# uncbiag/OAI_analysis_2

Hardware: NVIDIA B200
Metric: knee volumes/sec (seg+ICON reg+warp) (higher is better)
Workload: dtype fp16 operands / fp32 accumulate (tcgen05 kind::f16), the full-resolution decoder layers read fp16 hi+lo activations (dc2: skip input only; dc1); fp32 registration; fp64 warp coordinates

## Files before the change

include/oai_b200.h:

```cpp
#ifndef OAI_B200_H_
#define OAI_B200_H_

#include <stddef.h>
#include <stdint.h>

#if defined(__GNUC__)
#define OAI_API __attribute__((visibility("default")))
#else
#define OAI_API
#endif

#ifdef __cplusplus
extern "C" {
#endif

OAI_API const char* oai_last_error(void);
OAI_API int oai_version(void);
OAI_API long long oai_launch_count(void);


OAI_API int oai_conv3d_igemm(const void* src0, int c0, const void* src1, int c1, int NT, int D, int H, int W,
                     const void* wpack, size_t wpack_bytes, const float* bias, int cout, int pointwise, int relu,
                     int ab_format, void* out, long long obase, long long osN, long long osD, long long osH,
                     long long osW, int flags, void* stream);

OAI_API int oai_conv3d_igemm_region(const void* src0, int c0, const void* src1, int c1, int NT, int D, int H, int W,
                                    const void* wpack, size_t wpack_bytes, const float* bias, int cout, int pointwise,
                                    int relu, int ab_format, void* out, long long obase, long long osN, long long osD,
                                    long long osH, long long osW, int flags, const int* region, void* stream);

OAI_API int oai_pack_convt2_weights(const float* w, int cout, int cin, int D, int H, int W, int ab_format, void* dst,
                                    size_t dst_bytes);
OAI_API int oai_convt2_igemm(const void* src, int cin, int NT, int D, int H, int W, const void* wpack,
                             size_t wpack_bytes, const float* bias, int cout, int relu, int ab_format, void* out,
                             const int* region, void* stream);

OAI_API int oai_conv3d_igemm_head(const void* src0, int c0, const void* src1, int c1, int NT, int D, int H, int W,
                                  const void* wpack, size_t wpack_bytes, const float* bias, int ab_format, int ncls,
                                  const float* head_w, const float* head_b, float* out, const int* vol_dims,
                                  const int* geom, int tile0, const int* crop_zyx, int out_mode, int flags,
                                  void* stream);

OAI_API int oai_conv3d_igemm_plan(int D, int H, int W, int c0, int c1, int cout, int pointwise, int flags, int* plan);

OAI_API int oai_pack_conv_weights(const float* w, int cout, int c0, int c1, int D, int H, int W, int pointwise, int ab_format,
                          int flags, void* dst, size_t dst_bytes);

OAI_API int oai_conv3d_igemm_plan_ex(int D, int H, int W, int c0, int c1, int cout, int pointwise, int terms, int flags,
                                     int* plan);
OAI_API int oai_pack_conv_weights_ex(const float* w, int cout, int c0, int c1, int D, int H, int W, int pointwise,
                                     int terms, int ab_format, int flags, void* dst, size_t dst_bytes);
OAI_API int oai_conv3d_igemm_ex(const void* src0, int c0, const void* src1, int c1, int in_split, int NT, int D, int H,
                                int W, const void* wpack, size_t wpack_bytes, const float* bias, int cout,
                                int pointwise, int relu, int ab_format, int terms, void* out, int out_split, int flags,
                                const int* region, void* stream);

OAI_API int oai_conv_overflow_count(long long* count, int reset, void* stream);

// ... 193 lines not shown
```

oai_analysis_2_b200/csrc/api_conv.cu:

```cuda
#include "../../include/oai_b200.h"
#include "api_common.h"
#include "conv_api.h"
#include "conv_igemm.cuh"

#include <cuda_bf16.h>
#include <cuda_fp16.h>

#include <cstring>
#include <vector>

namespace oai {

cudaError_t conv_igemm_launch(const ConvIgemmParams& p, const CUtensorMap& tm0, const CUtensorMap& tm1, int num_sms,
                              cudaStream_t stream);
cudaError_t conv_overflow_count(unsigned int* count, bool reset, cudaStream_t stream);

namespace {

constexpr int kFlagForcePerTap = 1;
constexpr int kFlagBaseOffFormula = 2;
constexpr int kFlagForceKd1 = 4;
constexpr int kFlagNoFastPath = 8;
constexpr int kFlagWideN = 16;
constexpr int kFlagWideRows = 32;
constexpr int kFlagNoPingPong = 128;
constexpr int kFlagOneKhRow = 64;
constexpr size_t kSmemBudget = 232448 - 1024 - 48 * 8 - 2112 - 2048;

struct Chunk {
  int src, cc, wsel, dup;
};

struct Plan {
  int mode, kd_per_block, R, Rd, up_groups, nhalf, cph, nblk, nch, k16, row_bytes, TW, TH, n_wbuf, n_astage;
  int nkh;
  int pingpong;
  int stationary;
  uint32_t wblock_bytes, astage_bytes, astage_stride;
  Chunk chunks[kMaxChunks];
};

inline bool split_src(int terms, int src) {
  return terms == 2 || terms == 3 || (terms == 4 && src == 1) || (terms == 5 && src == 0);
}

int build_chunks(const ConvSpec& s, Plan* pl) {
  int n = 0;
  const int cs[2] = {s.c0, s.c1};
  for (int src = 0; src < 2; ++src) {
// ... 274 lines not shown
                const int v = ck.cc + j;
                if (v >= (ck.dup ? 2 * csrc : csrc)) break;
                const int ci = cbase + (ck.dup ? v % csrc : v);
                const uint16_t h = wrow[static_cast<size_t>(ci) * ktaps + tap];
                memcpy(blk + swz_off(r, j, pl.row_bytes), &h, 2);
              }
            }
          }
      }
  return 0;
}

int conv_run(const ConvSpec& s, const ConvLaunch& a, cudaStream_t st) {
  const int D = s.D, H = s.H, W = s.W, c0 = s.c0, c1 = s.c1, cout = s.cout;
  const bool kh_shared = (s.flags & kConvFlagKhShared) != 0;
  int d_lo = 0, d_cnt = D, h_lo = 0, h_cnt = H, w_lo = 0, w_cnt = W;
  if (a.region) {
    d_lo = a.region[0]; d_cnt = a.region[1]; h_lo = a.region[2]; h_cnt = a.region[3];
    OAI_REQUIRE(d_lo >= 0 && d_cnt >= 1 && d_lo + d_cnt <= D && h_lo >= 0 && h_cnt >= 1 && h_lo + h_cnt <= H,
                "conv: region [%d,+%d)x[%d,+%d) outside %dx%d", d_lo, d_cnt, h_lo, h_cnt, D, H);
  }
  if (a.w_cnt) {
    w_lo = a.w_lo; w_cnt = a.w_cnt;
    OAI_REQUIRE(kh_shared, "conv: a w range needs a layer packed for kh-shared mode");
    OAI_REQUIRE(w_lo >= 0 && w_cnt >= 1 && w_lo + w_cnt <= W, "conv: w range [%d,+%d) outside W=%d", w_lo, w_cnt, W);
  }
  int tw = 32, ntile = 0;
  if (kh_shared)
    for (int t = 32; t >= 8; t /= 2) {
      if (t > W || 128 / t > H) continue;
      const int n = ((w_cnt + t - 1) / t) * ((h_cnt + 128 / t - 1) / (128 / t));
      if (ntile == 0 || n < ntile) { ntile = n; tw = t; }
    }
  Plan pl;
  if (make_plan(s, &pl, d_cnt, tw)) return 1;
  int tile_h_lo = h_lo, nph = (h_cnt + pl.TH - 1) / pl.TH, npw = (w_cnt + pl.TW - 1) / pl.TW;
  if (!kh_shared) {
    tile_h_lo = h_lo / pl.TH * pl.TH;
    nph = (h_lo + h_cnt + pl.TH - 1) / pl.TH - h_lo / pl.TH;
    npw = W / pl.TW;
  }
  const HeadFuse* head = a.head;
  OAI_REQUIRE(a.src0 && a.wpack && a.bias, "conv: null pointer");
  OAI_REQUIRE(!head || (pl.cph == 64 && pl.nhalf == 1), "conv head: the fused head needs a 64-channel layer");
  OAI_REQUIRE((c1 == 0) == (a.src1 == nullptr), "conv: src1/c1 mismatch");
  const size_t need = plan_wpack_bytes(pl);
  OAI_REQUIRE(a.wpack_bytes == need, "conv: packed weights are %zu bytes, geometry needs %zu", a.wpack_bytes, need);
// ... 8 lines not shown
  p.TW = pl.TW; p.TH = pl.TH; p.R = pl.R;
  p.cout = pl.cph; p.nhalf = pl.nhalf;
  p.nchunks = pl.nch; p.k16_steps = pl.k16; p.row_bytes = pl.row_bytes;
  for (int c = 0; c < pl.nch; ++c) {
    p.chunk_src[c] = static_cast<uint8_t>(pl.chunks[c].src);
    p.chunk_cc[c] = static_cast<uint16_t>(pl.chunks[c].cc);
  }
  p.mode = pl.mode; p.kd_per_block = pl.kd_per_block; p.nblk = pl.nblk / pl.nkh;
  p.wblock_bytes = pl.wblock_bytes * pl.nkh; p.n_wbuf = pl.n_wbuf; p.n_astage = pl.n_astage;
  p.nkh = pl.nkh;
  p.acc_pingpong = pl.pingpong;
  p.w_stationary = pl.stationary;
  p.astage_bytes = pl.astage_bytes; p.astage_stride = pl.astage_stride;
  p.ab_format = s.fmt; p.relu = a.relu;
  p.base_off_mode = (s.flags & kFlagBaseOffFormula) ? 1 : 0;
  p.no_fast_path = (s.flags & kFlagNoFastPath) ? 1 : 0;
  p.wpack = static_cast<const uint8_t*>(a.wpack);
  p.bias = a.bias;
  p.out = a.out;
  p.obase = a.obase; p.osN = a.osN; p.osD = a.osD; p.osH = a.osH; p.osW = a.osW;
  p.out_split = a.out_split; p.out_lo_off = a.out_lo_off;
  p.d_lo = d_lo; p.d_cnt = d_cnt; p.h_lo = tile_h_lo; p.nph = nph; p.w_lo = kh_shared ? w_lo : 0; p.npw = npw;
  p.Rd = pl.Rd; p.up_groups = pl.up_groups;
  p.nunits = a.NT * ((d_cnt + pl.Rd - 1) / pl.Rd) * (nph * npw) * pl.up_groups * pl.nhalf;
  if (pl.mode == kModeUp2) {
    const long long vox = a.osW / 2;
    for (int t = 0; t < 8; ++t)
      p.tap_off[t] = ((static_cast<long long>(t >> 2) * 2 * H + ((t >> 1) & 1)) * 2 * W + (t & 1)) * vox;
  }
  if (head) p.head = *head;

  OAI_REQUIRE(pl.mode != kModeUp2 || (c1 == 0 && !head), "conv: up2 mode takes one source and no fused head");
  const int bw = pl.mode == kModeRowShared ? 130 : pl.TW;
  const int bh = pl.mode == kModeKhShared ? pl.TH + 2 : pl.TH * pl.nkh;
  CUtensorMap tm0, tm1;
  if (make_act_tmap(&tm0, a.src0, s.split0 ? 2 * c0 : c0, W, H, D, a.NT, bw, bh, s.fmt, pl.row_bytes)) return 1;
  if (a.src1) {
    if (make_act_tmap(&tm1, a.src1, s.split1 ? 2 * c1 : c1, W, H, D, a.NT, bw, bh, s.fmt)) return 1;
  } else {
    tm1 = tm0;
  }
  ProfEntry* pe = nullptr;
  if (g_prof_on) {
    if (g_prof_used == g_prof.size()) {
      ProfEntry ne;
      if (cudaEventCreate(&ne.a) != cudaSuccess || cudaEventCreate(&ne.b) != cudaSuccess)
        return fail("conv profile: cannot create events");
// ... 174 lines not shown
  if (int rc = check_cuda(cudaEventSynchronize(g_prof[i].b), "conv profile: event sync")) return rc;
  float t = 0;
  if (int rc = check_cuda(cudaEventElapsedTime(&t, g_prof[i].a, g_prof[i].b), "conv profile: elapsed")) return rc;
  if (ms) *ms = t;
  if (flops) *flops = g_prof[i].flops;
  if (exec_flops) *exec_flops = g_prof[i].exec_flops;
  return 0;
}


extern "C" int oai_pack_convt2_weights(const float* w, int cout, int cin, int D, int H, int W, int ab_format,
                                       void* dst, size_t dst_bytes) {
  return conv_pack_weights(spec_of(D, H, W, cin, 0, cout, 2, ab_format, 0), w, dst, dst_bytes);
}

extern "C" int oai_convt2_igemm(const void* src, int cin, int NT, int D, int H, int W, const void* wpack,
                                size_t wpack_bytes, const float* bias, int cout, int relu, int ab_format, void* out,
                                const int* region, void* stream) {
  OAI_REQUIRE(out != nullptr, "convt2: null output");
  const long long c = cout;
  return conv_common(src, cin, nullptr, 0, NT, D, H, W, wpack, wpack_bytes, bias, cout, 2, relu, ab_format, out, 0,
                     8ll * D * H * W * c, 8ll * H * W * c, 4ll * W * c, 2 * c, 0, nullptr, region, stream);
}
```

oai_analysis_2_b200/csrc/conv_api.h:

```cpp
#pragma once
#include <cstddef>
#include <cuda_runtime.h>

#include "conv_igemm.cuh"

namespace oai {

constexpr int kConvFlagKhShared = 256;

struct ConvSpec {
  int D, H, W;
  int c0, c1;
  int split0, split1;
  int cout;
  int kind;
  int terms;
  int fmt;
  int flags;
};

struct ConvLaunch {
  const void* src0;
  const void* src1;
  int NT;
  const void* wpack;
  size_t wpack_bytes;
  const float* bias;
  int relu;
  void* out;
  long long obase, osN, osD, osH, osW;
  int out_split;
// ... 25 lines not shown
```

oai_analysis_2_b200/csrc/conv_igemm.cu:

```cuda
#include "conv_igemm.cuh"
#include "ptx.cuh"

#include <cuda_bf16.h>
#include <cuda_fp16.h>

namespace oai {

namespace {

constexpr int kThreads = 384;
constexpr int kEpiGroups = 2;
constexpr int kTmemCols = 512;

__device__ unsigned int g_fp16_overflow = 0;

struct BlockInfo {
  int c, kh, kw, kdlo, nkd;
  int ns;
};

__device__ __forceinline__ BlockInfo decode_block(const ConvIgemmParams& p, int b) {
  BlockInfo bi;
  if (p.mode == kModeRowShared) {
    bi.c = p.nkh == 3 ? b : b / 3;
// ... 26 lines not shown
  } else {
    bi.c = b;
    bi.kh = 1;
    bi.kw = 1;
    bi.kdlo = 1;
    bi.nkd = 1;
  }
  bi.ns = (p.mode == kModeUp2) ? p.R : bi.nkd;
  return bi;
}

struct UnitInfo {
  int n, d0, h0, w0, nh;
  int tg;
  int rd;
  int ra;
};

__device__ __forceinline__ UnitInfo decode_unit(const ConvIgemmParams& p, int u) {
  UnitInfo ui;
  const int npw = p.npw;
  const int np = npw * p.nph, ndg = (p.d_cnt + p.Rd - 1) / p.Rd;
  if (p.w_stationary) {
    const int per_key = np * ndg * p.NT;
    const int key = u / per_key;
    u -= key * per_key;
    ui.tg = key % p.up_groups;
    ui.nh = key / p.up_groups;
  } else {
    ui.nh = u % p.nhalf;
    u /= p.nhalf;
    ui.tg = u % p.up_groups;
    u /= p.up_groups;
  }
  const int patch = u % np;
  u /= np;
  ui.d0 = p.d_lo + (u % ndg) * p.Rd;
  ui.n = u / ndg;
  ui.h0 = min(p.h_lo + (patch / npw) * p.TH, p.H - p.TH);
  ui.w0 = min(p.w_lo + (patch % npw) * p.TW, p.W - p.TW);
  ui.rd = min(p.Rd, p.d_lo + p.d_cnt - ui.d0);
  ui.ra = (p.mode == kModeUp2) ? p.R : ui.rd;
  return ui;
}

template <int FMT>
__device__ __forceinline__ uint32_t pack2(float a, float b) {
  if (FMT == 0) {
    __half2 h = __floats2half2_rn(a, b);
// ... 1 lines not shown
  }
  __nv_bfloat162 h = __floats2bfloat162_rn(a, b);
  return *reinterpret_cast<uint32_t*>(&h);
}

__device__ __forceinline__ void st_global_256(void* p, const uint32_t* v) {
  asm volatile("st.global.v8.b32 [%0], {%1,%2,%3,%4,%5,%6,%7,%8};" ::"l"(p), "r"(v[0]), "r"(v[1]), "r"(v[2]), "r"(v[3]),
               "r"(v[4]), "r"(v[5]), "r"(v[6]), "r"(v[7])
               : "memory");
}

template <int FMT>
__device__ __forceinline__ uint32_t pack2_residual(float a, float b, uint32_t hi) {
  if (FMT == 0) {
    const float2 h = __half22float2(*reinterpret_cast<const __half2*>(&hi));
    return pack2<FMT>(a - h.x, b - h.y);
  }
  const float2 h = __bfloat1622float2(*reinterpret_cast<const __nv_bfloat162*>(&hi));
  return pack2<FMT>(a - h.x, b - h.y);
}

template <int FMT, bool RELU, bool SPLIT>
__device__ __forceinline__ void epi_store_chunk(uint32_t (&v)[32], uint32_t sbias, uint16_t* dst, long long lo_off,
                                                float& amax) {
  uint32_t o[16];
#pragma unroll
  for (int i = 0; i < 8; ++i) {
    const float4 b4 = lds_f4(sbias + 16 * i);
    float x0 = __uint_as_float(v[4 * i]) + b4.x, x1 = __uint_as_float(v[4 * i + 1]) + b4.y;
    float x2 = __uint_as_float(v[4 * i + 2]) + b4.z, x3 = __uint_as_float(v[4 * i + 3]) + b4.w;
    if (RELU) {
      x0 = fmaxf(x0, 0.f); x1 = fmaxf(x1, 0.f); x2 = fmaxf(x2, 0.f); x3 = fmaxf(x3, 0.f);
    }
    amax = fmaxf(amax, fmaxf(fmaxf(fabsf(x0), fabsf(x1)), fmaxf(fabsf(x2), fabsf(x3))));
    o[2 * i] = pack2<FMT>(x0, x1);
    o[2 * i + 1] = pack2<FMT>(x2, x3);
    if (SPLIT) {
      v[4 * i] = __float_as_uint(x0); v[4 * i + 1] = __float_as_uint(x1);
      v[4 * i + 2] = __float_as_uint(x2); v[4 * i + 3] = __float_as_uint(x3);
    }
  }
  st_global_256(dst, o);
  st_global_256(dst + 16, o + 8);
  if (SPLIT) {
#pragma unroll
    for (int i = 0; i < 16; ++i)
      o[i] = pack2_residual<FMT>(__uint_as_float(v[2 * i]), __uint_as_float(v[2 * i + 1]), o[i]);
    st_global_256(dst + lo_off, o);
    st_global_256(dst + lo_off + 16, o + 8);
  }
}

template <int FMT, bool RELU, bool SPLIT>
__device__ __forceinline__ void epi_store_acc(uint32_t t_acc, int nb, uint32_t sbias, uint16_t* dst, long long lo_off,
                                              uint64_t* acc_empty_bar, int lane, float& amax) {
  for (int j = 0; j < nb; ++j) {
    uint32_t v[32];
    tmem_ld_32x32(t_acc + j * 32, v);
    tmem_ld_wait();
    if (j + 1 == nb) {
      tc_fence_before();
      __syncwarp();
      if (lane == 0) mbar_arrive(acc_empty_bar);
    }
    epi_store_chunk<FMT, RELU, SPLIT>(v, sbias + j * 128, dst + j * 32, lo_off, amax);
  }
}

template <int NC>
__device__ __forceinline__ void head_dot(const uint32_t (&v)[32], uint32_t sbias, uint32_t sw, float (&acc)[8],
                                         int ncls = NC) {
#pragma unroll
  for (int i = 0; i < 8; ++i) {
    const float4 b4 = lds_f4(sbias + 16 * i);
    const float f0 = fmaxf(__uint_as_float(v[4 * i]) + b4.x, 0.f), f1 = fmaxf(__uint_as_float(v[4 * i + 1]) + b4.y, 0.f);
    const float f2 = fmaxf(__uint_as_float(v[4 * i + 2]) + b4.z, 0.f), f3 = fmaxf(__uint_as_float(v[4 * i + 3]) + b4.w, 0.f);
#pragma unroll
    for (int k = 0; k < NC; ++k)
      if (k < ncls) {
        const float4 w4 = lds_f4(sw + k * 256 + 16 * i);
        acc[k] = fmaf(f3, w4.w, fmaf(f2, w4.z, fmaf(f1, w4.y, fmaf(f0, w4.x, acc[k]))));
      }
  }
}


struct IssueConsts {
  uint32_t kw_step, b_kw, desc_hi32, idesc_1, idesc_step, tap16, cout;
// ... 358 lines not shown
    const int per_rt = max(1, 256 / p.cout);
#define OAI_ISSUE(NKW, K16N, PER) \
  mma_issuer_fast<NKW, K16N, PER, 1>(p, tmem_base, abuf, wbuf, wstride, full_a, empty_a, full_w, empty_w, acc_full, acc_empty)
#define OAI_ISSUE_GENERAL() \
  mma_issuer_general(p, tmem_base, abuf, wbuf, wstride, full_a, empty_a, full_w, empty_w, acc_full, acc_empty)
    if (general) OAI_ISSUE_GENERAL();
    else if (nkw_rt == 3 && p.k16_steps == 4 && per_rt == 4) OAI_ISSUE(3, 4, 4);
    else if (nkw_rt == 3 && p.k16_steps == 2 && per_rt == 4 && p.nkh == 3)
      mma_issuer_fast<3, 2, 4, 3>(p, tmem_base, abuf, wbuf, wstride, full_a, empty_a, full_w, empty_w, acc_full, acc_empty);
    else if (nkw_rt == 3 && p.k16_steps == 2 && per_rt == 4) OAI_ISSUE(3, 2, 4);
    else if (nkw_rt == 1 && p.k16_steps == 4 && per_rt == 4) OAI_ISSUE(1, 4, 4);
    else if (nkw_rt == 1 && p.k16_steps == 4 && per_rt == 2) OAI_ISSUE(1, 4, 2);
    else if (nkw_rt == 1 && p.k16_steps == 4 && per_rt == 1) OAI_ISSUE(1, 4, 1);
    else OAI_ISSUE_GENERAL();
#undef OAI_ISSUE_GENERAL
#undef OAI_ISSUE
  } else if (warp >= 4) {
    const int q = warp & 3;
    const int eg = (warp - 4) >> 2;
    const int epi_variant = (p.ab_format ? 4 : 0) + (p.out_split ? 2 : 0) + (p.relu ? 1 : 0);
    const uint32_t s_bias_addr = smem_u32(s_bias), s_head_addr = smem_u32(s_head);
    const int m = q * 32 + lane;
    const int th = m / p.TW, tw = m % p.TW;
    uint32_t ub0 = 0, ub1 = 0;
    int half = 0;
    const uint32_t tmem_base0 = tmem_base;
    uint64_t* const acc_full0 = acc_full;
    uint64_t* const acc_empty0 = acc_empty;
    uint16_t* out = reinterpret_cast<uint16_t*>(p.out);
    float amax = 0.f;
    for (int u = blockIdx.x; u < p.nunits; u += gridDim.x) {
      const UnitInfo ui = decode_unit(p, u);
      const int ab = half * p.R;
      const uint32_t tmem_base = tmem_base0 + static_cast<uint32_t>(ab * p.cout);
      uint64_t* const acc_full = acc_full0 + ab;
      uint64_t* const acc_empty = acc_empty0 + ab;
      const int this_half = half;
      const uint32_t use_bits = this_half ? ub1 : ub0;
      if (p.acc_pingpong) half ^= 1;
      const long long off0 = p.obase + ui.n * p.osN + (ui.h0 + th) * p.osH + (ui.w0 + tw) * p.osW +
                             static_cast<long long>(ui.nh) * p.cout;
      for (int a = 0; a < ui.ra; ++a) {
        if (((ab + a) % kEpiGroups) != eg) continue;
        mbar_wait(&acc_full[a], (use_bits >> a) & 1u, 600 + a);
        tc_fence_after();
        if (p.head.enabled) {
          const HeadFuse& hd = p.head;
          const int z = ui.d0 + a - hd.od, y = ui.h0 + th - hd.oh, x = ui.w0 + tw - hd.ow;
          const bool row_in = z >= 0 && z < hd.ed;
          const bool mine = row_in && y >= 0 && y < hd.eh && x >= 0 && x < hd.ew;
          if (__any_sync(0xffffffffu, mine)) {
            float acc[8];
#pragma unroll
            for (int k = 0; k < 8; ++k) acc[k] = 0.f;
            for (int j = 0; j < 2; ++j) {
              uint32_t v[32];
              tmem_ld_32x32(tmem_base + (static_cast<uint32_t>(q * 32) << 16) +
                                static_cast<uint32_t>(a * p.cout + j * 32), v);
              tmem_ld_wait();
              const uint32_t sbj = s_bias_addr + static_cast<uint32_t>(ui.nh * p.cout + j * 32) * 4u;
              const uint32_t swj = s_head_addr + static_cast<uint32_t>(j * 32) * 4u;
              switch (hd.ncls) {
                case 1: head_dot<1>(v, sbj, swj, acc); break;
                case 2: head_dot<2>(v, sbj, swj, acc); break;
// ... 12 lines not shown
                const size_t o = (static_cast<size_t>(gz) * hd.VH + gy) * hd.VW + gx;
                const size_t cls_stride = static_cast<size_t>(hd.VD) * hd.VH * hd.VW;
#pragma unroll
                for (int k = 0; k < 8; ++k) {
                  if (k >= hd.ncls) break;
                  float r = 0.f;
                  if (!shell) {
                    const float logit = acc[k] + s_head[hd.ncls * 64 + k];
                    r = hd.out_mode == 2 ? logit : 1.f / (1.f + __expf(-logit));
                    if (hd.out_mode == 1) r = r > 0.5f ? 1.f : 0.f;
                  }
                  hd.out[k * cls_stride + o] = r;
                }
              }
            }
          }
        } else {
          uint16_t* dst = (p.mode == kModeUp2) ? out + off0 + ui.d0 * p.osD + p.tap_off[ui.tg * p.R + a]
                                               : out + off0 + (ui.d0 + a) * p.osD;
          const uint32_t sb = s_bias_addr + static_cast<uint32_t>(ui.nh * p.cout) * 4u;
          const uint32_t t_acc = tmem_base + (static_cast<uint32_t>(q * 32) << 16) + static_cast<uint32_t>(a * p.cout);
          const int nb = p.cout / 32;
          switch (epi_variant) {
            case 0: epi_store_acc<0, false, false>(t_acc, nb, sb, dst, p.out_lo_off, &acc_empty[a], lane, amax); break;
            case 1: epi_store_acc<0, true, false>(t_acc, nb, sb, dst, p.out_lo_off, &acc_empty[a], lane, amax); break;
            case 2: epi_store_acc<0, false, true>(t_acc, nb, sb, dst, p.out_lo_off, &acc_empty[a], lane, amax); break;
            case 3: epi_store_acc<0, true, true>(t_acc, nb, sb, dst, p.out_lo_off, &acc_empty[a], lane, amax); break;
            case 4: epi_store_acc<1, false, false>(t_acc, nb, sb, dst, p.out_lo_off, &acc_empty[a], lane, amax); break;
            case 5: epi_store_acc<1, true, false>(t_acc, nb, sb, dst, p.out_lo_off, &acc_empty[a], lane, amax); break;
            case 6: epi_store_acc<1, false, true>(t_acc, nb, sb, dst, p.out_lo_off, &acc_empty[a], lane, amax); break;
            default: epi_store_acc<1, true, true>(t_acc, nb, sb, dst, p.out_lo_off, &acc_empty[a], lane, amax); break;
          }
          continue;
        }
        tc_fence_before();
        __syncwarp();
        if (lane == 0) mbar_arrive(&acc_empty[a]);
      }
      if (this_half) ub1 = use_bits ^ ((1u << ui.ra) - 1u);
      else ub0 = use_bits ^ ((1u << ui.ra) - 1u);
    }
    if (p.ab_format == 0 && !(amax <= 65504.f)) atomicAdd(&g_fp16_overflow, 1u);
  }

  tc_fence_before();
  __syncthreads();
  if (warp == 2) {
    tc_fence_after();
    tmem_dealloc(tmem_base, kTmemCols);
  }
}


static size_t conv_igemm_smem_bytes(const ConvIgemmParams& p) {
// ... 32 lines not shown
```

oai_analysis_2_b200/csrc/conv_igemm.cuh:

```cuda
#pragma once
#include <cstdint>
#include <cuda.h>
#include <cuda_runtime.h>

namespace oai {

constexpr int kMaxChunks = 48;

enum ConvMode : int {
  kModeRowShared = 0,
  kModePerTap = 1,
  kModePointwise = 2,
  kModeUp2 = 3,
  kModeKhShared = 4,
};

struct HeadFuse {
  int enabled;
  int ncls, out_mode;
  const float* w;
  const float* b;
  float* out;
  int VD, VH, VW;
  int ed, eh, ew, od, oh, ow, gh, gw, tile0;
// ... 4 lines not shown
  int NT, D, H, W;
  int TW, TH;
  int R;
  int Rd;
  int up_groups;
  long long tap_off[8];
  int d_lo, d_cnt;
  int h_lo, nph;
  int w_lo, npw;
  int cout;
  int nhalf;
  int nchunks;
  uint16_t chunk_cc[kMaxChunks];
  uint8_t chunk_src[kMaxChunks];
  int k16_steps;
  int row_bytes;
  int mode;
  int kd_per_block;
  int nblk;
  uint32_t wblock_bytes;
  int n_wbuf;
  int nkh;
  int w_stationary;
  int acc_pingpong;
  int n_astage;
  uint32_t astage_bytes;
  uint32_t astage_stride;
  int ab_format;
  int relu;
  int no_fast_path;
  int base_off_mode;
  const uint8_t* wpack;
  const float* bias;
  void* out;
  long long obase, osN, osD, osH, osW;
  int out_split;
  long long out_lo_off;
  int nunits;
  HeadFuse head;
};

}
```

oai_analysis_2_b200/csrc/seg_net.cu:

```cuda
#include "../../include/oai_b200.h"
#include "api_common.h"
#include "conv_api.h"
#include "seg_misc.cuh"

#include <nvtx3/nvToolsExt.h>

#include <algorithm>
#include <cmath>
#include <cstdlib>
#include <cstring>
#include <map>
#include <set>
#include <string>
#include <vector>

using namespace oai;

namespace {

struct LayerDef {
  const char* name;
  char kind;
  int cin, cout;
  int level;
// ... 31 lines not shown
  void* w = nullptr;
  size_t w_bytes = 0;
  float* bias = nullptr;
};

struct Box {
  int lo[3], hi[3];
};

}

struct oai_seg_handle {
  oai_seg_config cfg;
  int device;
  int tile[3], overlap[3];
  int terms[kNumLayers];
  int split[kNumTensors];
  PackedLayer layers[kNumLayers];
  float* stem_w = nullptr;
  float* head_w = nullptr;
  float* head_b = nullptr;
  bool has_region = false;
  Box region[kNumLayers];
};

namespace {

int dims_at(const oai_seg_handle* h, int level, int a) { return h->tile[a] >> level; }

size_t tensor_bytes(const oai_seg_handle* h, int t, int NT) {
  const TensorDef& d = kTensors[t];
  size_t n = static_cast<size_t>(NT) * dims_at(h, d.level, 0) * dims_at(h, d.level, 1) * dims_at(h, d.level, 2) *
             d.channels * 2 * (h->split[t] ? 2 : 1);
  return (n + 255) & ~size_t(255);
}

size_t plan_workspace(const oai_seg_handle* h, int NT, size_t* offs) {
  struct Live { size_t off, size; int last; };
  std::vector<Live> live;
  size_t peak = 0;
  for (int t = 0; t < kNumTensors; ++t) {
    const int birth = kTensors[t].birth;
    live.erase(std::remove_if(live.begin(), live.end(), [&](const Live& l) { return l.last < birth; }), live.end());
    std::sort(live.begin(), live.end(), [](const Live& a, const Live& b) { return a.off < b.off; });
    const size_t size = tensor_bytes(h, t, NT);
    size_t off = 0;
// ... 42 lines not shown
  const int ups[2][3] = {{DC3, DC4, DC5}, {DC6, DC7, DC8}};
  for (int i = 0; i < 2; ++i) {
    const int lvl = i + 1;
    const Box q = half(need, lvl);
    region[ups[i][0]] = q;
    region[ups[i][1]] = q;
    region[ups[i][2]] = dil(q, 1, lvl);
    need = dil(q, 2, lvl);
  }
  region[DC9] = half(need, 3);
}

struct NamedTensor {
  const float* data;
  std::vector<long long> shape;
  long long numel;
};

bool w_halo_skip_disabled() {
  const char* e = getenv("OAI_B200_SEG_W_HALO");
  return e && e[0] == '0';
}

int device_copy(const void* host, size_t bytes, void** dev) {
  if (int rc = check_cuda(cudaMalloc(dev, bytes), "seg_create: cudaMalloc")) return rc;
  return check_cuda(cudaMemcpy(*dev, host, bytes, cudaMemcpyHostToDevice), "seg_create: cudaMemcpy");
}

}

extern "C" int oai_seg_needed_regions(const int* tile_zyx, const int* overlap_zyx, int* boxes) {
  OAI_REQUIRE(tile_zyx && overlap_zyx && boxes, "seg_needed_regions: null pointer");
  Box region[kNumLayers];
  needed_regions(tile_zyx, overlap_zyx, region);
  for (int l = 0; l < kNumLayers; ++l)
    for (int a = 0; a < 3; ++a) {
      boxes[l * 6 + a] = region[l].lo[a];
      boxes[l * 6 + 3 + a] = region[l].hi[a];
    }
  return 0;
}

extern "C" int oai_seg_layer_terms(int precision, int* terms17) {
  OAI_REQUIRE(terms17 != nullptr, "seg_layer_terms: null pointer");
  OAI_REQUIRE(precision >= OAI_SEG_PRECISION_FP16 && precision <= OAI_SEG_PRECISION_FP16X3,
              "seg_layer_terms: unknown precision %d", precision);
// ... 39 lines not shown
    OAI_REQUIRE(h->overlap[a] >= 0 && 2 * h->overlap[a] < h->tile[a],
                "seg_create: overlap_size must be smaller than half the patch size");
  }
  if (cfg->precision == OAI_SEG_PRECISION_CUSTOM) {
    for (int l = 0; l < kNumLayers; ++l) {
      h->terms[l] = l == 0 ? 1 : cfg->layer_terms[l];
      OAI_REQUIRE(h->terms[l] >= 1 && h->terms[l] <= 5 && (h->terms[l] < 4 || kLayers[l].c_first > 0),
                  "seg_create: layer_terms[%d]=%d", l, h->terms[l]);
    }
  } else if (oai_seg_layer_terms(cfg->precision, h->terms)) {
    return 1;
  }
  for (int t = 0; t < kNumTensors; ++t) {
    const int c = kTensors[t].consumers[0];
    const bool is_skip = t == T_SYN0 || t == T_SYN1 || t == T_SYN2;
    const int tm = c >= 0 ? h->terms[c] : 1;
    h->split[t] = tm == 2 || tm == 3 || (tm == 4 && is_skip) || (tm == 5 && !is_skip);
  }
  for (int i = 0; i < 3; ++i)
    if (h->split[kPoolOf[i][1]]) h->split[kPoolOf[i][0]] = 1;
  needed_regions(h->tile, h->overlap, h->region);
  h->has_region = h->overlap[0] || h->overlap[1] || h->overlap[2];
  const bool skip_w_halo = h->has_region && !w_halo_skip_disabled();

  std::set<std::string> consumed;
  auto take = [&](const std::string& key, std::initializer_list<long long> shape, const NamedTensor** out) -> int {
    auto it = sd.find(key);
    OAI_REQUIRE(it != sd.end(), "seg_create: missing key %s in state_dict", key.c_str());
    const NamedTensor& t = it->second;
    bool ok = t.shape.size() == shape.size() && t.data != nullptr;
    size_t i = 0;
    for (long long s : shape) ok = ok && t.shape[i++] == s;
    OAI_REQUIRE(ok, "seg_create: size mismatch for %s", key.c_str());
    *out = &t;
    consumed.insert(key);
    return 0;
  };
  const int ncls = cfg->n_classes;
  for (int l = 0; l < kNumLayers; ++l) {
    const LayerDef& L = kLayers[l];
    const std::string nm = L.name;
    const int k = L.kind == 'u' ? 2 : 3, taps = k * k * k, ci = L.cin, co = L.cout;
    const NamedTensor *w, *b = nullptr, *g = nullptr, *beta = nullptr, *mean = nullptr, *var = nullptr;
    if (L.kind == 'c') {
      if (take(nm + ".0.weight", {co, ci, k, k, k}, &w)) return 1;
    } else {
// ... 19 lines not shown
          const size_t src = L.kind == 'c' ? (static_cast<size_t>(o) * ci + i) * taps + t
                                           : (static_cast<size_t>(i) * co + o) * taps + (L.kind == 't' ? taps - 1 - t : t);
          wf[(static_cast<size_t>(o) * ci + i) * taps + t] = static_cast<float>(static_cast<double>(w->data[src]) * s);
        }
    }
    PackedLayer& P = h->layers[l];
    if (device_copy(bf.data(), bf.size() * sizeof(float), reinterpret_cast<void**>(&P.bias))) return 1;
    if (l == EC0) {
      std::vector<float> w27(27 * co);
      for (int t = 0; t < 27; ++t)
        for (int o = 0; o < co; ++o) w27[t * co + o] = wf[static_cast<size_t>(o) * 27 + t];
      if (device_copy(w27.data(), w27.size() * sizeof(float), reinterpret_cast<void**>(&h->stem_w))) return 1;
      continue;
    }
    ConvSpec& s = P.spec;
    s.D = dims_at(h, L.level, 0); s.H = dims_at(h, L.level, 1); s.W = dims_at(h, L.level, 2);
    s.c0 = L.c_first ? L.c_first : ci;
    s.c1 = ci - s.c0;
    s.cout = co;
    s.kind = L.kind == 'u' ? 2 : 0;
    s.terms = h->terms[l];
    s.fmt = cfg->ab_format;
    s.flags = (skip_w_halo && (l == DC2 || l == DC1) && s.W % 128 == 0) ? kConvFlagKhShared : 0;
    s.split0 = s.split1 = 0;
    ConvSpec ps = s;
    ps.split0 = s.terms == 2 || s.terms == 3 || s.terms == 5;
    ps.split1 = (s.terms == 2 || s.terms == 3 || s.terms == 4) && s.c1 > 0;
    P.w_bytes = conv_wpack_bytes(ps);
    OAI_REQUIRE(P.w_bytes > 0, "seg_create: layer %s: %s", L.name, oai_last_error());
    std::vector<uint8_t> img(P.w_bytes);
    if (conv_pack_weights(ps, wf.data(), img.data(), img.size())) return 1;
    if (device_copy(img.data(), img.size(), &P.w)) return 1;
  }
  {
    const NamedTensor *w0, *b0 = nullptr;
    if (take("dc0.weight", {ncls, 64, 1, 1, 1}, &w0)) return 1;
    if (cfg->bias && take("dc0.bias", {ncls}, &b0)) return 1;
    std::vector<float> hb(ncls, 0.f);
    if (b0) std::copy(b0->data, b0->data + ncls, hb.begin());
    if (device_copy(w0->data, static_cast<size_t>(ncls) * 64 * sizeof(float), reinterpret_cast<void**>(&h->head_w)) ||
        device_copy(hb.data(), ncls * sizeof(float), reinterpret_cast<void**>(&h->head_b)))
      return 1;
  }
  for (const auto& kv : sd)
    OAI_REQUIRE(consumed.count(kv.first), "seg_create: unexpected key %s in state_dict", kv.first.c_str());
  guard.h = nullptr;
// ... 76 lines not shown
    ConvLaunch a;
    a.src0 = buf(t0);
    a.src1 = t1 >= 0 ? buf(t1) : nullptr;
    a.NT = NT; a.wpack = P.w; a.wpack_bytes = P.w_bytes; a.bias = P.bias; a.relu = 1;
    a.out = buf(tout);
    a.obase = 0;
    a.out_split = h->split[tout];
    a.out_lo_off = L.cout;
    const long long cp = (a.out_split ? 2ll : 1ll) * L.cout;
    if (L.kind == 'u') {
      a.osN = 8ll * s.D * s.H * s.W * cp; a.osD = 8ll * s.H * s.W * cp; a.osH = 4ll * s.W * cp; a.osW = 2 * cp;
    } else {
      a.osN = 1ll * s.D * s.H * s.W * cp; a.osD = 1ll * s.H * s.W * cp; a.osH = 1ll * s.W * cp; a.osW = cp;
    }
    int region[4];
    a.region = nullptr;
    if (h->has_region && l >= DC9) {
      const Box& b = h->region[l];
      region[0] = b.lo[0]; region[1] = b.hi[0] - b.lo[0] + 1; region[2] = b.lo[1]; region[3] = b.hi[1] - b.lo[1] + 1;
      a.region = region;
    }
    a.head = nullptr;
    if (a.region && (s.flags & kConvFlagKhShared)) return conv_w_box(s, a, h->region[l].lo[2], h->region[l].hi[2]);
    return conv_run(s, a, st);
  };
  auto pool = [&](int i, int NT) -> int {
    const int tin = kPoolOf[i][0], tout = kPoolOf[i][1];
    const TensorDef& d = kTensors[tin];
    return maxpool2_launch(buf(tin), buf(tout), NT, dims_at(h, d.level, 0), dims_at(h, d.level, 1),
                           dims_at(h, d.level, 2), d.channels, h->split[tin], h->split[tout], fmt, st);
  };

  nvtxRangePushA("oai.seg_forward");
  int rc = 0;
  for (int t0 = 0; t0 < T && !rc; t0 += nb) {
    const int NT = std::min(nb, T - t0);
    StemParams sp;
    sp.vol = vol; sp.VD = vol_dims[0]; sp.VH = vol_dims[1]; sp.VW = vol_dims[2];
    sp.td = geom[0]; sp.th = geom[1]; sp.tw = geom[2];
    sp.ed = geom[3]; sp.eh = geom[4]; sp.ew = geom[5];
    sp.od = geom[6]; sp.oh = geom[7]; sp.ow = geom[8];
    sp.gh = geom[10]; sp.gw = geom[11];
    sp.tile0 = t0; sp.ntiles = NT; sp.c0 = 32; sp.w = h->stem_w; sp.b = h->layers[EC0].bias; sp.out = buf(T_E0);
    sp.fmt = fmt; sp.out_split = h->split[T_E0];
    rc = stem_launch(sp, st)
         || conv(EC1, NT, T_E0, -1, T_SYN0)
// ... 33 lines not shown
```

oai_analysis_2_b200/ops.py:

```python
import ctypes
import math

import numpy as np
import torch

from ._lib import c_double, c_float, c_int, c_ll, c_size, check, lib, ptr, stream_ptr

FLAG_FORCE_PER_TAP = 1
FLAG_BASE_OFF_FORMULA = 2
FLAG_FORCE_KD1 = 4
FLAG_NO_FAST_PATH = 8
FLAG_WIDE_N = 16

_DT16 = {0: torch.float16, 1: torch.bfloat16}


def conv_plan(D, H, W, c0, c1, cout, pointwise=False, flags=0):
    plan = (c_int * 9)()
    check(lib.oai_conv3d_igemm_plan(D, H, W, c0, c1, cout, int(pointwise), flags, plan), "conv plan")
    keys = ("mode", "kd_per_block", "R", "nhalf", "cout_per_half", "nblk", "wblock_bytes", "nchunks", "row_bytes")
    return dict(zip(keys, list(plan)))


def pack_conv_weights(w, c0, c1, D, H, W, pointwise=False, ab_format=0, flags=0, device="cuda"):
# ... 516 lines not shown
def conv3d_igemm_head(src0, wpack, bias, head_w, head_b, out, geom, tile0, crop_zyx, out_mode=0, ab_format=0,
                      flags=0):
    NT, D, H, W, c0 = src0.shape
    ncls = head_w.shape[0]
    dims = np.asarray(out.shape[1:], dtype=np.int32)
    crop = np.asarray(crop_zyx, dtype=np.int32)
    check(lib.oai_conv3d_igemm_head(ptr(src0), c0, None, 0, NT, D, H, W, ptr(wpack), c_size(wpack.numel()), ptr(bias),
                                    ab_format, ncls, ptr(head_w), ptr(head_b), ptr(out), ptr(dims), ptr(geom), tile0,
                                    ptr(crop), out_mode, flags, stream_ptr()), "conv3d_igemm_head")
    return out


def pack_convt2_weights(w, D, H, W, ab_format=0, device="cuda"):
    w = np.ascontiguousarray(w.detach().cpu().numpy() if hasattr(w, "detach") else w, dtype=np.float32)
    cout, cin = w.shape[:2]
    pl = conv_plan(D, H, W, cin, 0, cout, 2)
    nbytes = pl["nhalf"] * pl["kd_per_block"] * pl["nblk"] * pl["wblock_bytes"]
    dst = np.zeros(nbytes, dtype=np.uint8)
    check(lib.oai_pack_convt2_weights(ptr(w), cout, cin, D, H, W, ab_format, ptr(dst), c_size(nbytes)),
          "pack convt2 weights")
    return torch.from_numpy(dst).to(device)


def convt2_igemm(src, wpack, bias, cout, relu=True, ab_format=0, region=None, out=None):
    NT, D, H, W, cin = src.shape
    assert src.is_contiguous()
    if out is None:
        out = torch.empty((NT, 2 * D, 2 * H, 2 * W, cout), dtype=_DT16[ab_format], device=src.device)
    reg = None if region is None else np.asarray(region, dtype=np.int32)
    check(lib.oai_convt2_igemm(ptr(src), cin, NT, D, H, W, ptr(wpack), c_size(wpack.numel()), ptr(bias), cout,
                               int(relu), ab_format, ptr(out), ptr(reg), stream_ptr()), "convt2_igemm")
    return out


def intensity_window(vol, perc_lo=0.1, perc_hi=99.9, out_min=0.0, out_max=1.0, out=None, return_window=False):
    assert vol.dtype == torch.float32 and vol.is_contiguous()
    if out is None:
        out = torch.empty_like(vol)
    nbytes = int(lib.oai_intensity_window_workspace())
    ws = _scratch_buf(vol.device, "window", nbytes)
    check(lib.oai_intensity_window(ptr(vol), c_ll(vol.numel()), ctypes.c_double(perc_lo), ctypes.c_double(perc_hi),
                                   c_float(out_min), c_float(out_max), ptr(out), ptr(ws), c_size(nbytes),
                                   stream_ptr()), "intensity_window")
    if return_window:
        w = (ctypes.c_double * 2)()
        check(lib.oai_intensity_window_result(ptr(ws), w, stream_ptr()), "intensity_window_result")
        return out, (w[0], w[1])
    return out


def mc_table():
    t = np.zeros((256, 64, 32), dtype=np.uint8)
# ... 127 lines not shown
```

Measured before the change: 10.17.

## Window weight-stationary up2 conv schedule and skip stores outside needed W range

For weight-stationary transposed-conv (up2) layers, units are reordered so that each group of tiles, sized to about 32 MiB of activation data across the grid, is swept over all weight keys before moving on. This aims to keep activations resident in L2 instead of re-streaming the whole input once per weight key. The epilogue also drops global stores and amax updates for output columns outside a requested W range, and DC3 now passes that W range when DC2 is kh-shared. The MMA work for those columns is still done, the unit index math gets more complex, and an env var and flag can turn the windowing off.

```diff
diff --git a/include/oai_b200.h b/include/oai_b200.h
--- a/include/oai_b200.h
+++ b/include/oai_b200.h
@@ -34,6 +34,9 @@
 OAI_API int oai_convt2_igemm(const void* src, int cin, int NT, int D, int H, int W, const void* wpack,
                              size_t wpack_bytes, const float* bias, int cout, int relu, int ab_format, void* out,
                              const int* region, void* stream);
+OAI_API int oai_convt2_igemm_box(const void* src, int cin, int NT, int D, int H, int W, const void* wpack,
+                                 size_t wpack_bytes, const float* bias, int cout, int relu, int ab_format, void* out,
+                                 const int* box, int flags, void* stream);
 
 OAI_API int oai_conv3d_igemm_head(const void* src0, int c0, const void* src1, int c1, int NT, int D, int H, int W,
                                   const void* wpack, size_t wpack_bytes, const float* bias, int ab_format, int ncls,
diff --git a/oai_analysis_2_b200/csrc/api_conv.cu b/oai_analysis_2_b200/csrc/api_conv.cu
--- a/oai_analysis_2_b200/csrc/api_conv.cu
+++ b/oai_analysis_2_b200/csrc/api_conv.cu
@@ -6,6 +6,7 @@
 #include <cuda_bf16.h>
 #include <cuda_fp16.h>
 
+#include <algorithm>
 #include <cstring>
 #include <vector>
 
@@ -25,6 +26,7 @@
 constexpr int kFlagWideRows = 32;
 constexpr int kFlagNoPingPong = 128;
 constexpr int kFlagOneKhRow = 64;
+constexpr size_t kUp2WindowBytes = 32u << 20;
 constexpr size_t kSmemBudget = 232448 - 1024 - 48 * 8 - 2112 - 2048;
 
 struct Chunk {
@@ -345,7 +347,7 @@
   }
   if (a.w_cnt) {
     w_lo = a.w_lo; w_cnt = a.w_cnt;
-    OAI_REQUIRE(kh_shared, "conv: a w range needs a layer packed for kh-shared mode");
+    OAI_REQUIRE(kh_shared || s.kind == 2, "conv: a w range needs a k2s2 layer or one packed for kh-shared mode");
     OAI_REQUIRE(w_lo >= 0 && w_cnt >= 1 && w_lo + w_cnt <= W, "conv: w range [%d,+%d) outside W=%d", w_lo, w_cnt, W);
   }
   int tw = 32, ntile = 0;
@@ -400,7 +402,17 @@
   p.out_split = a.out_split; p.out_lo_off = a.out_lo_off;
   p.d_lo = d_lo; p.d_cnt = d_cnt; p.h_lo = tile_h_lo; p.nph = nph; p.w_lo = kh_shared ? w_lo : 0; p.npw = npw;
   p.Rd = pl.Rd; p.up_groups = pl.up_groups;
-  p.nunits = a.NT * ((d_cnt + pl.Rd - 1) / pl.Rd) * (nph * npw) * pl.up_groups * pl.nhalf;
+  const int ntiles = a.NT * ((d_cnt + pl.Rd - 1) / pl.Rd) * (nph * npw);
+  p.nunits = ntiles * pl.up_groups * pl.nhalf;
+  p.win_tiles = ntiles;
+  if (pl.mode == kModeUp2 && pl.stationary && !(s.flags & kConvFlagNoUp2Window)) {
+    const int grid = std::min(p.nunits, num_sms());
+    const size_t tile_bytes = static_cast<size_t>(pl.nblk) * pl.astage_bytes;
+    const int k = std::max(1, static_cast<int>(kUp2WindowBytes / (tile_bytes * grid)));
+    p.win_tiles = std::min(ntiles, k * grid);
+  }
+  p.st_w_lo = pl.mode == kModeUp2 ? w_lo : 0;
+  p.st_w_hi = pl.mode == kModeUp2 ? w_lo + w_cnt : W;
   if (pl.mode == kModeUp2) {
     const long long vox = a.osW / 2;
     for (int t = 0; t < 8; ++t)
@@ -621,3 +633,17 @@
   return conv_common(src, cin, nullptr, 0, NT, D, H, W, wpack, wpack_bytes, bias, cout, 2, relu, ab_format, out, 0,
                      8ll * D * H * W * c, 8ll * H * W * c, 4ll * W * c, 2 * c, 0, nullptr, region, stream);
 }
+
+extern "C" int oai_convt2_igemm_box(const void* src, int cin, int NT, int D, int H, int W, const void* wpack,
+                                    size_t wpack_bytes, const float* bias, int cout, int relu, int ab_format, void* out,
+                                    const int* box, int flags, void* stream) {
+  OAI_REQUIRE(out != nullptr && box != nullptr, "convt2 box: null pointer");
+  OAI_REQUIRE(flags == 0 || flags == kConvFlagNoUp2Window, "convt2 box: flags=%d (0 or %d)", flags, kConvFlagNoUp2Window);
+  const long long c = cout;
+  ConvLaunch a;
+  a.src0 = src; a.src1 = nullptr; a.NT = NT; a.wpack = wpack; a.wpack_bytes = wpack_bytes; a.bias = bias; a.relu = relu;
+  a.out = out; a.obase = 0; a.osN = 8ll * D * H * W * c; a.osD = 8ll * H * W * c; a.osH = 4ll * W * c; a.osW = 2 * c;
+  a.out_split = 0; a.out_lo_off = 0; a.region = box; a.w_lo = box[4]; a.w_cnt = box[5]; a.head = nullptr;
+  OAI_REQUIRE(a.w_cnt >= 1, "convt2 box: w_cnt=%d", a.w_cnt);
+  return conv_run(spec_of(D, H, W, cin, 0, cout, 2, ab_format, flags), a, static_cast<cudaStream_t>(stream));
+}
diff --git a/oai_analysis_2_b200/csrc/conv_api.h b/oai_analysis_2_b200/csrc/conv_api.h
--- a/oai_analysis_2_b200/csrc/conv_api.h
+++ b/oai_analysis_2_b200/csrc/conv_api.h
@@ -7,6 +7,7 @@
 namespace oai {
 
 constexpr int kConvFlagKhShared = 256;
+constexpr int kConvFlagNoUp2Window = 512;
 
 struct ConvSpec {
   int D, H, W;
diff --git a/oai_analysis_2_b200/csrc/conv_igemm.cu b/oai_analysis_2_b200/csrc/conv_igemm.cu
--- a/oai_analysis_2_b200/csrc/conv_igemm.cu
+++ b/oai_analysis_2_b200/csrc/conv_igemm.cu
@@ -72,9 +72,13 @@
   const int npw = p.npw;
   const int np = npw * p.nph, ndg = (p.d_cnt + p.Rd - 1) / p.Rd;
   if (p.w_stationary) {
-    const int per_key = np * ndg * p.NT;
-    const int key = u / per_key;
-    u -= key * per_key;
+    const int ntiles = np * ndg * p.NT, nkeys = p.nhalf * p.up_groups;
+    const int win = u / (p.win_tiles * nkeys);
+    const int t0 = win * p.win_tiles;
+    const int wt = min(p.win_tiles, ntiles - t0);
+    u -= t0 * nkeys;
+    const int key = u / wt;
+    u = t0 + u - key * wt;
     ui.tg = key % p.up_groups;
     ui.nh = key / p.up_groups;
   } else {
@@ -122,8 +126,9 @@
 
 template <int FMT, bool RELU, bool SPLIT>
 __device__ __forceinline__ void epi_store_chunk(uint32_t (&v)[32], uint32_t sbias, uint16_t* dst, long long lo_off,
-                                                float& amax) {
+                                                bool live, float& amax) {
   uint32_t o[16];
+  float m = 0.f;
 #pragma unroll
   for (int i = 0; i < 8; ++i) {
     const float4 b4 = lds_f4(sbias + 16 * i);
@@ -132,7 +137,7 @@
     if (RELU) {
       x0 = fmaxf(x0, 0.f); x1 = fmaxf(x1, 0.f); x2 = fmaxf(x2, 0.f); x3 = fmaxf(x3, 0.f);
     }
-    amax = fmaxf(amax, fmaxf(fmaxf(fabsf(x0), fabsf(x1)), fmaxf(fabsf(x2), fabsf(x3))));
+    m = fmaxf(m, fmaxf(fmaxf(fabsf(x0), fabsf(x1)), fmaxf(fabsf(x2), fabsf(x3))));
     o[2 * i] = pack2<FMT>(x0, x1);
     o[2 * i + 1] = pack2<FMT>(x2, x3);
     if (SPLIT) {
@@ -140,6 +145,8 @@
       v[4 * i + 2] = __float_as_uint(x2); v[4 * i + 3] = __float_as_uint(x3);
     }
   }
+  if (!live) return;
+  amax = fmaxf(amax, m);
   st_global_256(dst, o);
   st_global_256(dst + 16, o + 8);
   if (SPLIT) {
@@ -153,7 +160,7 @@
 
 template <int FMT, bool RELU, bool SPLIT>
 __device__ __forceinline__ void epi_store_acc(uint32_t t_acc, int nb, uint32_t sbias, uint16_t* dst, long long lo_off,
-                                              uint64_t* acc_empty_bar, int lane, float& amax) {
+                                              uint64_t* acc_empty_bar, int lane, bool live, float& amax) {
   for (int j = 0; j < nb; ++j) {
     uint32_t v[32];
     tmem_ld_32x32(t_acc + j * 32, v);
@@ -163,7 +170,7 @@
       __syncwarp();
       if (lane == 0) mbar_arrive(acc_empty_bar);
     }
-    epi_store_chunk<FMT, RELU, SPLIT>(v, sbias + j * 128, dst + j * 32, lo_off, amax);
+    epi_store_chunk<FMT, RELU, SPLIT>(v, sbias + j * 128, dst + j * 32, lo_off, live, amax);
   }
 }
 
@@ -568,6 +575,7 @@
     const uint32_t s_bias_addr = smem_u32(s_bias), s_head_addr = smem_u32(s_head);
     const int m = q * 32 + lane;
     const int th = m / p.TW, tw = m % p.TW;
+    const int st_w_lo = p.st_w_lo, st_w_hi = p.st_w_hi;
     uint32_t ub0 = 0, ub1 = 0;
     int half = 0;
     const uint32_t tmem_base0 = tmem_base;
@@ -586,6 +594,7 @@
       if (p.acc_pingpong) half ^= 1;
       const long long off0 = p.obase + ui.n * p.osN + (ui.h0 + th) * p.osH + (ui.w0 + tw) * p.osW +
                              static_cast<long long>(ui.nh) * p.cout;
+      const bool live = ui.w0 + tw >= st_w_lo && ui.w0 + tw < st_w_hi;
       for (int a = 0; a < ui.ra; ++a) {
         if (((ab + a) % kEpiGroups) != eg) continue;
         mbar_wait(&acc_full[a], (use_bits >> a) & 1u, 600 + a);
@@ -644,14 +653,14 @@
           const uint32_t t_acc = tmem_base + (static_cast<uint32_t>(q * 32) << 16) + static_cast<uint32_t>(a * p.cout);
           const int nb = p.cout / 32;
           switch (epi_variant) {
-            case 0: epi_store_acc<0, false, false>(t_acc, nb, sb, dst, p.out_lo_off, &acc_empty[a], lane, amax); break;
-            case 1: epi_store_acc<0, true, false>(t_acc, nb, sb, dst, p.out_lo_off, &acc_empty[a], lane, amax); break;
-            case 2: epi_store_acc<0, false, true>(t_acc, nb, sb, dst, p.out_lo_off, &acc_empty[a], lane, amax); break;
-            case 3: epi_store_acc<0, true, true>(t_acc, nb, sb, dst, p.out_lo_off, &acc_empty[a], lane, amax); break;
-            case 4: epi_store_acc<1, false, false>(t_acc, nb, sb, dst, p.out_lo_off, &acc_empty[a], lane, amax); break;
-            case 5: epi_store_acc<1, true, false>(t_acc, nb, sb, dst, p.out_lo_off, &acc_empty[a], lane, amax); break;
-            case 6: epi_store_acc<1, false, true>(t_acc, nb, sb, dst, p.out_lo_off, &acc_empty[a], lane, amax); break;
-            default: epi_store_acc<1, true, true>(t_acc, nb, sb, dst, p.out_lo_off, &acc_empty[a], lane, amax); break;
+            case 0: epi_store_acc<0, false, false>(t_acc, nb, sb, dst, p.out_lo_off, &acc_empty[a], lane, live, amax); break;
+            case 1: epi_store_acc<0, true, false>(t_acc, nb, sb, dst, p.out_lo_off, &acc_empty[a], lane, live, amax); break;
+            case 2: epi_store_acc<0, false, true>(t_acc, nb, sb, dst, p.out_lo_off, &acc_empty[a], lane, live, amax); break;
+            case 3: epi_store_acc<0, true, true>(t_acc, nb, sb, dst, p.out_lo_off, &acc_empty[a], lane, live, amax); break;
+            case 4: epi_store_acc<1, false, false>(t_acc, nb, sb, dst, p.out_lo_off, &acc_empty[a], lane, live, amax); break;
+            case 5: epi_store_acc<1, true, false>(t_acc, nb, sb, dst, p.out_lo_off, &acc_empty[a], lane, live, amax); break;
+            case 6: epi_store_acc<1, false, true>(t_acc, nb, sb, dst, p.out_lo_off, &acc_empty[a], lane, live, amax); break;
+            default: epi_store_acc<1, true, true>(t_acc, nb, sb, dst, p.out_lo_off, &acc_empty[a], lane, live, amax); break;
           }
           continue;
         }
diff --git a/oai_analysis_2_b200/csrc/conv_igemm.cuh b/oai_analysis_2_b200/csrc/conv_igemm.cuh
--- a/oai_analysis_2_b200/csrc/conv_igemm.cuh
+++ b/oai_analysis_2_b200/csrc/conv_igemm.cuh
@@ -50,6 +50,7 @@
   int n_wbuf;
   int nkh;
   int w_stationary;
+  int win_tiles;
   int acc_pingpong;
   int n_astage;
   uint32_t astage_bytes;
@@ -64,6 +65,7 @@
   long long obase, osN, osD, osH, osW;
   int out_split;
   long long out_lo_off;
+  int st_w_lo, st_w_hi;
   int nunits;
   HeadFuse head;
 };
diff --git a/oai_analysis_2_b200/csrc/seg_net.cu b/oai_analysis_2_b200/csrc/seg_net.cu
--- a/oai_analysis_2_b200/csrc/seg_net.cu
+++ b/oai_analysis_2_b200/csrc/seg_net.cu
@@ -77,6 +77,7 @@
   float* head_b = nullptr;
   bool has_region = false;
   Box region[kNumLayers];
+  bool up2_window = true;
 };
 
 namespace {
@@ -165,6 +166,11 @@
   return e && e[0] == '0';
 }
 
+bool up2_window_disabled() {
+  const char* e = getenv("OAI_B200_SEG_UP2_WINDOW");
+  return e && e[0] == '0';
+}
+
 int device_copy(const void* host, size_t bytes, void** dev) {
   if (int rc = check_cuda(cudaMalloc(dev, bytes), "seg_create: cudaMalloc")) return rc;
   return check_cuda(cudaMemcpy(*dev, host, bytes, cudaMemcpyHostToDevice), "seg_create: cudaMemcpy");
@@ -250,6 +256,7 @@
   needed_regions(h->tile, h->overlap, h->region);
   h->has_region = h->overlap[0] || h->overlap[1] || h->overlap[2];
   const bool skip_w_halo = h->has_region && !w_halo_skip_disabled();
+  h->up2_window = !up2_window_disabled();
 
   std::set<std::string> consumed;
   auto take = [&](const std::string& key, std::initializer_list<long long> shape, const NamedTensor** out) -> int {
@@ -315,6 +322,7 @@
     s.terms = h->terms[l];
     s.fmt = cfg->ab_format;
     s.flags = (skip_w_halo && (l == DC2 || l == DC1) && s.W % 128 == 0) ? kConvFlagKhShared : 0;
+    if (L.kind == 'u' && !h->up2_window) s.flags |= kConvFlagNoUp2Window;
     s.split0 = s.split1 = 0;
     ConvSpec ps = s;
     ps.split0 = s.terms == 2 || s.terms == 3 || s.terms == 5;
@@ -437,6 +445,10 @@
     }
     a.head = nullptr;
     if (a.region && (s.flags & kConvFlagKhShared)) return conv_w_box(s, a, h->region[l].lo[2], h->region[l].hi[2]);
+    if (a.region && l == DC3 && h->up2_window && (h->layers[DC2].spec.flags & kConvFlagKhShared)) {
+      a.w_lo = h->region[l].lo[2];
+      a.w_cnt = h->region[l].hi[2] - h->region[l].lo[2] + 1;
+    }
     return conv_run(s, a, st);
   };
   auto pool = [&](int i, int NT) -> int {
diff --git a/oai_analysis_2_b200/ops.py b/oai_analysis_2_b200/ops.py
--- a/oai_analysis_2_b200/ops.py
+++ b/oai_analysis_2_b200/ops.py
@@ -562,12 +562,17 @@
     return torch.from_numpy(dst).to(device)
 
 
-def convt2_igemm(src, wpack, bias, cout, relu=True, ab_format=0, region=None, out=None):
+def convt2_igemm(src, wpack, bias, cout, relu=True, ab_format=0, region=None, out=None, flags=0):
     NT, D, H, W, cin = src.shape
     assert src.is_contiguous()
     if out is None:
         out = torch.empty((NT, 2 * D, 2 * H, 2 * W, cout), dtype=_DT16[ab_format], device=src.device)
     reg = None if region is None else np.asarray(region, dtype=np.int32)
+    if reg is not None and reg.size == 6:
+        check(lib.oai_convt2_igemm_box(ptr(src), cin, NT, D, H, W, ptr(wpack), c_size(wpack.numel()), ptr(bias), cout,
+                                       int(relu), ab_format, ptr(out), ptr(reg), flags, stream_ptr()), "convt2_igemm")
+        return out
+    assert flags == 0, "flags go with a six-entry region"
     check(lib.oai_convt2_igemm(ptr(src), cin, NT, D, H, W, ptr(wpack), c_size(wpack.numel()), ptr(bias), cout,
                                int(relu), ab_format, ptr(out), ptr(reg), stream_ptr()), "convt2_igemm")
     return out
```

Result: no change. 10.22, median of 6 (+0.5%).
